# saidwivedi/TokenHMR

Measured on NVIDIA H100. Metric: images/sec (256x192) at bs=64 per GPU, full TokenHMR forward, higher is better.
Workload: dtype f16 operands / f32 accumulate

## Files before the change

### tokenhmr_b200/_build.py

```python
from __future__ import annotations

import hashlib
import os
import subprocess
import sys
from pathlib import Path

PKG_DIR = Path(__file__).resolve().parent
CSRC = PKG_DIR / "csrc"
LIB_PATH = PKG_DIR / "libtokenhmr_b200.so"
STAMP = PKG_DIR / ".libtokenhmr_b200.stamp"
PROBE_SRC = PKG_DIR.parent / "tests" / "csrc" / "kernel_probe.cu"
PROBE_PATH = PKG_DIR.parent / "tests" / "libthmr_probe.so"
PROBE_STAMP = PKG_DIR.parent / "tests" / ".libthmr_probe.stamp"
GEMM_PROBE_SRC = PKG_DIR.parent / "tests" / "csrc" / "gemm_probe.cu"
GEMM_PROBE_PATH = PKG_DIR.parent / "tests" / "libthmr_gemm_probe.so"
GEMM_PROBE_STAMP = PKG_DIR.parent / "tests" / ".libthmr_gemm_probe.stamp"
HEAD_PROBE_SRC = PKG_DIR.parent / "tests" / "csrc" / "head_train_probe.cu"
HEAD_PROBE_PATH = PKG_DIR.parent / "tests" / "libthmr_head_train_probe.so"
HEAD_PROBE_STAMP = PKG_DIR.parent / "tests" / ".libthmr_head_train_probe.stamp"

NVCC_FLAGS = [
    "-gencode", "arch=compute_90a,code=sm_90a",
    "-lineinfo", "-O3", "-std=c++17",
    "--expt-relaxed-constexpr",
    "-Xcompiler", "-fPIC", "-shared",
]
PROBE_FLAGS = ["-Xcompiler", "-fvisibility=hidden"]


def _nvcc() -> str:
    for cand in (os.environ.get("NVCC"), "/usr/local/cuda/bin/nvcc", "nvcc"):
        if cand and (os.path.isabs(cand) and os.path.exists(cand) or not os.path.isabs(cand)):
            return cand
    return "nvcc"


def source_hash(probe: bool = False) -> str:
    h = hashlib.sha256()
    files = sorted(CSRC.glob("*.cu")) + sorted(CSRC.glob("*.cuh")) + sorted((PKG_DIR.parent / "include").glob("*.h"))
    if probe:
        files += sorted(PROBE_SRC.parent.glob("*.cu"))
    for f in files:
        h.update(f.name.encode())
        h.update(f.read_bytes())
    h.update(" ".join(NVCC_FLAGS + (PROBE_FLAGS if probe else [])).encode())
    return h.hexdigest()


def _compile(src: Path, out: Path, stamp: Path, flags: list, want: str, force: bool, verbose: bool) -> Path:
    if not force and out.exists() and stamp.exists() and stamp.read_text().strip() == want:
        return out
    cmd = [_nvcc(), *flags, "-o", str(out), str(src)]
    if verbose:
        cmd.insert(1, "-Xptxas=-v")
        print(" ".join(cmd), file=sys.stderr)
    res = subprocess.run(cmd, capture_output=True, text=True)
    if res.returncode != 0:
        raise RuntimeError(f"nvcc failed ({res.returncode}):\n{res.stdout}\n{res.stderr}")
    if verbose:
        print(res.stderr, file=sys.stderr)
    stamp.write_text(want)
    return out


def build_probe(force: bool = False, verbose: bool = False) -> Path:
    for src, out, stamp in ((GEMM_PROBE_SRC, GEMM_PROBE_PATH, GEMM_PROBE_STAMP),
                            (HEAD_PROBE_SRC, HEAD_PROBE_PATH, HEAD_PROBE_STAMP)):
        if src.exists():
            _compile(src, out, stamp, NVCC_FLAGS + PROBE_FLAGS, source_hash(probe=True), force, verbose)
    return _compile(PROBE_SRC, PROBE_PATH, PROBE_STAMP, NVCC_FLAGS + PROBE_FLAGS, source_hash(probe=True), force,
                    verbose)


def build(force: bool = False, verbose: bool = False) -> Path:
    path = _compile(CSRC / "tokenhmr_b200.cu", LIB_PATH, STAMP, NVCC_FLAGS, source_hash(), force, verbose)
    if PROBE_SRC.exists():
        build_probe(force, verbose)
    return path


if __name__ == "__main__":
    print(build(force="--force" in sys.argv, verbose="-v" in sys.argv))
```

### tokenhmr_b200/csrc/attention_mma.cuh

```cuda
#pragma once
#include "common.cuh"
#include "ptx.cuh"

namespace thmr {

constexpr int kAttTokens = 192;
constexpr int kAttHeadDim = 80;
constexpr int kAttPitch = 88;
constexpr int kAttWarps = 6;
constexpr int kAttThreads = 32 * kAttWarps;
constexpr uint32_t kAttMatBytes = kAttTokens * kAttPitch * 2;
constexpr uint32_t kAttSmemBytes = 3 * kAttMatBytes;

struct AttnParams {
  const __half* qkv;
  int ldq;
  int num_problems;
  int heads;
  float scale_log2e;
  __half* out;
  int ldo;
  float* dbg_s;
  unsigned long long* stamp;
};

__device__ __forceinline__ float fast_exp2(float x) {
  float y;
  asm("ex2.approx.ftz.f32 %0, %1;" : "=f"(y) : "f"(x));
  return y;
}
__device__ __forceinline__ void ldmatrix_x4(uint32_t (&r)[4], uint32_t addr) {
  asm volatile("ldmatrix.sync.aligned.m8n8.x4.shared.b16 {%0, %1, %2, %3}, [%4];"
               : "=r"(r[0]), "=r"(r[1]), "=r"(r[2]), "=r"(r[3]) : "r"(addr));
}
__device__ __forceinline__ void ldmatrix_x4_trans(uint32_t (&r)[4], uint32_t addr) {
  asm volatile("ldmatrix.sync.aligned.m8n8.x4.trans.shared.b16 {%0, %1, %2, %3}, [%4];"
               : "=r"(r[0]), "=r"(r[1]), "=r"(r[2]), "=r"(r[3]) : "r"(addr));
}
__device__ __forceinline__ void mma_16816(float (&d)[4], const uint32_t (&a)[4], uint32_t b0, uint32_t b1) {
  asm volatile("mma.sync.aligned.m16n8k16.row.col.f32.f16.f16.f32 {%0, %1, %2, %3}, {%4, %5, %6, %7}, {%8, %9}, "
               "{%0, %1, %2, %3};"
               : "+f"(d[0]), "+f"(d[1]), "+f"(d[2]), "+f"(d[3])
               : "r"(a[0]), "r"(a[1]), "r"(a[2]), "r"(a[3]), "r"(b0), "r"(b1));
}
__device__ __forceinline__ uint32_t pack_half2(float a, float b) {
  __half2 h = __floats2half2_rn(a, b);
  return *reinterpret_cast<uint32_t*>(&h);
}

template <bool DBG>
__global__ void __launch_bounds__(kAttThreads, 2) vit_attention_kernel(const AttnParams p) {
  extern __shared__ __align__(16) uint8_t att_smem[];
  const uint32_t aQ = smem_u32(att_smem), aK = aQ + kAttMatBytes, aV = aK + kAttMatBytes;
  const int prob = blockIdx.x;
  const int b = prob / p.heads, h = prob % p.heads;
  const int warp = threadIdx.x >> 5, lane = threadIdx.x & 31;

  pdl_launch_dependents();
  stamp_start(p.stamp);
  pdl_wait();

  const __half* src = p.qkv + static_cast<size_t>(b) * kAttTokens * p.ldq;
  for (int i = threadIdx.x; i < 3 * kAttTokens * 10; i += kAttThreads) {
    const int m = i / (kAttTokens * 10), r = (i / 10) % kAttTokens, c = i % 10;
    const __half* g = src + static_cast<size_t>(r) * p.ldq + (m * p.heads + h) * kAttHeadDim + c * 8;
    const uint32_t s = aQ + m * kAttMatBytes + (r * kAttPitch + c * 8) * 2;
    asm volatile("cp.async.cg.shared.global [%0], [%1], 16;" ::"r"(s), "l"(g) : "memory");
  }
  asm volatile("cp.async.commit_group;\n\tcp.async.wait_group 0;" ::: "memory");
  __syncthreads();

  const int g = lane >> 2, t4 = lane & 3;
  for (int tile = warp; tile < kAttTokens / 16; tile += kAttWarps) {
    const int r0 = tile * 16;
    uint32_t qa[5][4];
#pragma unroll
    for (int kk = 0; kk < 5; ++kk)
      ldmatrix_x4(qa[kk], aQ + ((r0 + (lane & 15)) * kAttPitch + kk * 16 + 8 * (lane >> 4)) * 2);
    float s[24][4];
#pragma unroll
    for (int nt = 0; nt < 24; ++nt) s[nt][0] = s[nt][1] = s[nt][2] = s[nt][3] = 0.f;
#pragma unroll
    for (int np = 0; np < 12; ++np) {
#pragma unroll
      for (int kk = 0; kk < 5; ++kk) {
        uint32_t kb[4];
        ldmatrix_x4(kb, aK + ((np * 16 + (lane & 7) + 8 * (lane >> 4)) * kAttPitch + kk * 16 + 8 * ((lane >> 3) & 1)) * 2);
        mma_16816(s[2 * np], qa[kk], kb[0], kb[1]);
        mma_16816(s[2 * np + 1], qa[kk], kb[2], kb[3]);
      }
    }
    if (DBG) {
      float* d = p.dbg_s + (static_cast<size_t>(prob) * kAttTokens + r0 + g) * kAttTokens + 2 * t4;
#pragma unroll
      for (int nt = 0; nt < 24; ++nt) {
        *reinterpret_cast<float2*>(d + nt * 8) = make_float2(s[nt][0], s[nt][1]);
        *reinterpret_cast<float2*>(d + 8 * kAttTokens + nt * 8) = make_float2(s[nt][2], s[nt][3]);
      }
    }
    float mx0 = -INFINITY, mx1 = -INFINITY;
#pragma unroll
    for (int nt = 0; nt < 24; ++nt) {
      mx0 = fmaxf(mx0, fmaxf(s[nt][0], s[nt][1]));
      mx1 = fmaxf(mx1, fmaxf(s[nt][2], s[nt][3]));
    }
#pragma unroll
    for (int off = 1; off <= 2; off <<= 1) {
      mx0 = fmaxf(mx0, __shfl_xor_sync(0xffffffffu, mx0, off));
      mx1 = fmaxf(mx1, __shfl_xor_sync(0xffffffffu, mx1, off));
    }
    const float mo0 = mx0 * p.scale_log2e, mo1 = mx1 * p.scale_log2e;
    float sum0 = 0.f, sum1 = 0.f;
    uint32_t pa[12][4];
#pragma unroll
    for (int nt = 0; nt < 24; ++nt) {
      const float e0 = fast_exp2(fmaf(s[nt][0], p.scale_log2e, -mo0));
      const float e1 = fast_exp2(fmaf(s[nt][1], p.scale_log2e, -mo0));
      const float e2 = fast_exp2(fmaf(s[nt][2], p.scale_log2e, -mo1));
      const float e3 = fast_exp2(fmaf(s[nt][3], p.scale_log2e, -mo1));
      sum0 += e0 + e1;
      sum1 += e2 + e3;
      pa[nt >> 1][(nt & 1) * 2 + 0] = pack_half2(e0, e1);
      pa[nt >> 1][(nt & 1) * 2 + 1] = pack_half2(e2, e3);
    }
#pragma unroll
    for (int off = 1; off <= 2; off <<= 1) {
      sum0 += __shfl_xor_sync(0xffffffffu, sum0, off);
      sum1 += __shfl_xor_sync(0xffffffffu, sum1, off);
    }
    float o[10][4];
#pragma unroll
    for (int dt = 0; dt < 10; ++dt) o[dt][0] = o[dt][1] = o[dt][2] = o[dt][3] = 0.f;
#pragma unroll
    for (int ks = 0; ks < 12; ++ks) {
#pragma unroll
      for (int dp = 0; dp < 5; ++dp) {
        uint32_t vb[4];
        ldmatrix_x4_trans(vb, aV + ((ks * 16 + (lane & 7) + 8 * ((lane >> 3) & 1)) * kAttPitch + dp * 16 + 8 * (lane >> 4)) * 2);
        mma_16816(o[2 * dp], pa[ks], vb[0], vb[1]);
        mma_16816(o[2 * dp + 1], pa[ks], vb[2], vb[3]);
      }
    }
    const float inv0 = 1.0f / sum0, inv1 = 1.0f / sum1;
    __half* out = p.out + (static_cast<size_t>(b) * kAttTokens + r0 + g) * p.ldo + h * kAttHeadDim + 2 * t4;
#pragma unroll
    for (int dt = 0; dt < 10; ++dt) {
      *reinterpret_cast<uint32_t*>(out + dt * 8) = pack_half2(o[dt][0] * inv0, o[dt][1] * inv0);
      *reinterpret_cast<uint32_t*>(out + 8 * static_cast<size_t>(p.ldo) + dt * 8) = pack_half2(o[dt][2] * inv1, o[dt][3] * inv1);
    }
  }
}

struct AttnPlan {
  AttnParams p;
  int grid;
};

inline int attention_make_plan(const __half* qkv, int ld_qkv, int B, int heads, __half* out, int ldo, float* dbg_s,
                               AttnPlan* plan) {
  THMR_CHECK(B > 0 && heads > 0, "attention: bad shape");
  THMR_CHECK(ld_qkv >= 3 * heads * kAttHeadDim, "attention: qkv pitch %d < %d", ld_qkv, 3 * heads * kAttHeadDim);
  THMR_CHECK((reinterpret_cast<uintptr_t>(qkv) & 15) == 0 && ld_qkv % 8 == 0, "attention: qkv pointer/pitch alignment");
  THMR_CHECK(ldo % 2 == 0 && (reinterpret_cast<uintptr_t>(out) & 3) == 0, "attention: output alignment");
  plan->p.qkv = qkv;
  plan->p.ldq = ld_qkv;
  plan->p.num_problems = B * heads;
  plan->p.heads = heads;
  plan->p.scale_log2e = 1.4426950408889634f / sqrtf(static_cast<float>(kAttHeadDim));
  plan->p.out = out;
  plan->p.ldo = ldo;
  plan->p.dbg_s = dbg_s;
  plan->p.stamp = nullptr;
  plan->grid = plan->p.num_problems;
  return THMR_OK;
}

template <bool DBG>
inline int attention_launch_t(const AttnPlan& plan, cudaStream_t st) {
  static bool configured = false;
  if (!configured) {
    THMR_CUDA(cudaFuncSetAttribute(vit_attention_kernel<DBG>, cudaFuncAttributeMaxDynamicSharedMemorySize, kAttSmemBytes));
    configured = true;
  }
  THMR_CUDA(launch_pdl(vit_attention_kernel<DBG>, plan.grid, kAttThreads, kAttSmemBytes, st, plan.p));
  return THMR_OK;
}

inline int attention_dispatch(const AttnPlan& plan, cudaStream_t st) {
  return plan.p.dbg_s ? attention_launch_t<true>(plan, st) : attention_launch_t<false>(plan, st);
}

}
```

### tokenhmr_b200/csrc/ptx.cuh

```cuda
#pragma once
#include <cuda.h>
#include <cuda_fp16.h>
#include <cuda_runtime.h>
#include <stdint.h>

namespace thmr {

__device__ unsigned int g_pipeline_timeout = 0;
constexpr uint32_t kSpinLimit = 1u << 24;

__device__ __forceinline__ uint32_t smem_u32(const void* p) {
  return static_cast<uint32_t>(__cvta_generic_to_shared(p));
}

__device__ __forceinline__ void sts_f32x2(uint32_t a, float x, float y) {
  asm volatile("st.shared.v2.f32 [%0], {%1, %2};" ::"r"(a), "f"(x), "f"(y));
}
__device__ __forceinline__ float4 lds_f32x4(uint32_t a) {
  float4 v;
  asm volatile("ld.shared.v4.f32 {%0, %1, %2, %3}, [%4];" : "=f"(v.x), "=f"(v.y), "=f"(v.z), "=f"(v.w) : "r"(a));
  return v;
}
__device__ __forceinline__ void sts_f32(uint32_t a, float x) { asm volatile("st.shared.f32 [%0], %1;" ::"r"(a), "f"(x)); }
__device__ __forceinline__ void sts_u32(uint32_t a, uint32_t x) { asm volatile("st.shared.b32 [%0], %1;" ::"r"(a), "r"(x)); }
__device__ __forceinline__ float lds_f32(uint32_t a) {
  float v;
  asm volatile("ld.shared.f32 %0, [%1];" : "=f"(v) : "r"(a));
  return v;
}
__device__ __forceinline__ void named_barrier_sync(uint32_t id, uint32_t threads) {
  asm volatile("bar.sync %0, %1;" ::"r"(id), "r"(threads) : "memory");
}

__device__ __forceinline__ unsigned long long globaltimer() {
  unsigned long long t;
  asm volatile("mov.u64 %0, %%globaltimer;" : "=l"(t));
  return t;
}
__device__ __forceinline__ uint32_t smid() {
  uint32_t s;
  asm volatile("mov.u32 %0, %%smid;" : "=r"(s));
  return s;
}

__device__ __forceinline__ uint32_t lane_id() {
  uint32_t l;
  asm volatile("mov.u32 %0, %%laneid;" : "=r"(l));
  return l;
}

__device__ __forceinline__ void mbar_init(uint64_t* bar, uint32_t count) {
  asm volatile("mbarrier.init.shared::cta.b64 [%0], %1;" ::"r"(smem_u32(bar)), "r"(count) : "memory");
}
__device__ __forceinline__ void fence_mbar_init() {
  asm volatile("fence.mbarrier_init.release.cluster;" ::: "memory");
}
__device__ __forceinline__ void fence_proxy_async_smem() {
  asm volatile("fence.proxy.async.shared::cta;" ::: "memory");
}
__device__ __forceinline__ void mbar_arrive(uint64_t* bar) {
  asm volatile("mbarrier.arrive.shared::cta.b64 _, [%0];" ::"r"(smem_u32(bar)) : "memory");
}
__device__ __forceinline__ void mbar_arrive_expect_tx(uint64_t* bar, uint32_t bytes) {
  asm volatile("mbarrier.arrive.expect_tx.shared::cta.b64 _, [%0], %1;" ::"r"(smem_u32(bar)), "r"(bytes)
               : "memory");
}
__device__ __forceinline__ bool mbar_try_wait(uint64_t* bar, uint32_t parity) {
  uint32_t ok;
  asm volatile(
      "{\n\t"
      ".reg .pred P;\n\t"
      "mbarrier.try_wait.parity.shared::cta.b64 P, [%1], %2;\n\t"
      "selp.u32 %0, 1, 0, P;\n\t"
      "}\n"
      : "=r"(ok)
      : "r"(smem_u32(bar)), "r"(parity)
      : "memory");
  return ok != 0;
}
__device__ __forceinline__ bool mbar_wait(uint64_t* bar, uint32_t parity) {
#pragma unroll 1
  for (uint32_t it = 0; it < kSpinLimit; ++it) {
    if (mbar_try_wait(bar, parity)) return true;
  }
  atomicExch(&g_pipeline_timeout, 1u);
  return false;
}

__device__ __forceinline__ uint32_t cluster_ctarank() {
  uint32_t r;
  asm volatile("mov.u32 %0, %%cluster_ctarank;" : "=r"(r));
  return r;
}
__device__ __forceinline__ void cluster_sync_all() {
  asm volatile("barrier.cluster.arrive.release;\n\tbarrier.cluster.wait.acquire;" ::: "memory");
}
__device__ __forceinline__ void mbar_arrive_cluster(uint64_t* bar, uint32_t cta) {
  asm volatile(
      "{\n\t"
      ".reg .b32 ra;\n\t"
      "mapa.shared::cluster.u32 ra, %0, %1;\n\t"
      "mbarrier.arrive.release.cluster.shared::cluster.b64 _, [ra];\n\t"
      "}\n" ::"r"(smem_u32(bar)),
      "r"(cta)
      : "memory");
}
__device__ __forceinline__ bool mbar_wait_cluster(uint64_t* bar, uint32_t parity) {
#pragma unroll 1
  for (uint32_t it = 0; it < kSpinLimit; ++it) {
    uint32_t ok;
    asm volatile(
        "{\n\t"
        ".reg .pred P;\n\t"
        "mbarrier.try_wait.parity.acquire.cluster.shared::cta.b64 P, [%1], %2;\n\t"
        "selp.u32 %0, 1, 0, P;\n\t"
        "}\n"
        : "=r"(ok)
        : "r"(smem_u32(bar)), "r"(parity)
        : "memory");
    if (ok) return true;
  }
  atomicExch(&g_pipeline_timeout, 1u);
  return false;
}

__device__ __forceinline__ void tma_prefetch_desc(const CUtensorMap* m) {
  asm volatile("prefetch.tensormap [%0];" ::"l"(reinterpret_cast<uint64_t>(m)) : "memory");
}
__device__ __forceinline__ void tma_load_2d(void* smem_dst, const CUtensorMap* m, uint64_t* bar, int32_t c0,
                                            int32_t c1) {
  asm volatile(
      "cp.async.bulk.tensor.2d.shared::cluster.global.mbarrier::complete_tx::bytes"
      " [%0], [%1, {%3, %4}], [%2];"
      :
      : "r"(smem_u32(smem_dst)), "l"(reinterpret_cast<uint64_t>(m)), "r"(smem_u32(bar)), "r"(c0), "r"(c1)
      : "memory");
}
__device__ __forceinline__ void tma_load_2d_mcast(void* smem_dst, const CUtensorMap* m, uint64_t* bar, int32_t c0,
                                                  int32_t c1, uint16_t cta_mask) {
  asm volatile(
      "cp.async.bulk.tensor.2d.shared::cluster.global.mbarrier::complete_tx::bytes.multicast::cluster"
      " [%0], [%1, {%3, %4}], [%2], %5;"
      :
      : "r"(smem_u32(smem_dst)), "l"(reinterpret_cast<uint64_t>(m)), "r"(smem_u32(bar)), "r"(c0), "r"(c1),
        "h"(cta_mask)
      : "memory");
}
__device__ __forceinline__ void tma_store_2d(const CUtensorMap* m, uint32_t smem_src, int32_t c0, int32_t c1) {
  asm volatile("cp.async.bulk.tensor.2d.global.shared::cta.bulk_group [%0, {%2, %3}], [%1];"
               :
               : "l"(reinterpret_cast<uint64_t>(m)), "r"(smem_src), "r"(c0), "r"(c1)
               : "memory");
}
__device__ __forceinline__ void tma_reduce_add_2d(const CUtensorMap* m, uint32_t smem_src, int32_t c0, int32_t c1) {
  asm volatile("cp.reduce.async.bulk.tensor.2d.global.shared::cta.add.tile.bulk_group [%0, {%2, %3}], [%1];"
               :
               : "l"(reinterpret_cast<uint64_t>(m)), "r"(smem_src), "r"(c0), "r"(c1)
               : "memory");
}
__device__ __forceinline__ void tma_store_commit() { asm volatile("cp.async.bulk.commit_group;" ::: "memory"); }
template <int N>
__device__ __forceinline__ void tma_store_wait_read() {
  asm volatile("cp.async.bulk.wait_group.read %0;" ::"n"(N) : "memory");
}
template <int N>
__device__ __forceinline__ void tma_store_wait() {
  asm volatile("cp.async.bulk.wait_group %0;" ::"n"(N) : "memory");
}

__device__ __forceinline__ uint64_t make_wgmma_desc_sw128(uint32_t saddr) {
  uint64_t d = 0;
  d |= static_cast<uint64_t>((saddr >> 4) & 0x3FFF);
  d |= static_cast<uint64_t>(1) << 16;
  d |= static_cast<uint64_t>(1024 >> 4) << 32;
  d |= static_cast<uint64_t>(1) << 62;
  return d;
}
__device__ __forceinline__ void wgmma_fence() { asm volatile("wgmma.fence.sync.aligned;" ::: "memory"); }
__device__ __forceinline__ void wgmma_commit() { asm volatile("wgmma.commit_group.sync.aligned;" ::: "memory"); }
template <int N>
__device__ __forceinline__ void wgmma_wait() {
  asm volatile("wgmma.wait_group.sync.aligned %0;" ::"n"(N) : "memory");
}
template <int N>
__device__ __forceinline__ void wgmma_fence_operand(float (&d)[N]) {
#pragma unroll
  for (int i = 0; i < N; ++i) asm volatile("" : "+f"(d[i])::"memory");
}

__device__ __forceinline__ void wgmma_m64n32k16(float (&d)[16], uint64_t da, uint64_t db, uint32_t scale_d) {
  asm volatile(
      "{\n\t.reg .pred p;\n\tsetp.ne.b32 p, %18, 0;\n\t"
      "wgmma.mma_async.sync.aligned.m64n32k16.f32.f16.f16 {%0, %1, %2, %3, %4, %5, %6, %7, %8, %9, %10, %11, %12, %13, %14, %15}, %16, %17, p, 1, 1, 0, 0;\n\t}\n"
      : "+f"(d[0]), "+f"(d[1]), "+f"(d[2]), "+f"(d[3]), "+f"(d[4]), "+f"(d[5]), "+f"(d[6]), "+f"(d[7]), "+f"(d[8]), "+f"(d[9]), "+f"(d[10]), "+f"(d[11]), "+f"(d[12]), "+f"(d[13]), "+f"(d[14]), "+f"(d[15])
      : "l"(da), "l"(db), "r"(scale_d));
}
__device__ __forceinline__ void wgmma_m64n64k16(float (&d)[32], uint64_t da, uint64_t db, uint32_t scale_d) {
  asm volatile(
      "{\n\t.reg .pred p;\n\tsetp.ne.b32 p, %34, 0;\n\t"
      "wgmma.mma_async.sync.aligned.m64n64k16.f32.f16.f16 {%0, %1, %2, %3, %4, %5, %6, %7, %8, %9, %10, %11, %12, %13, %14, %15, %16, %17, %18, %19, %20, %21, %22, %23, %24, %25, %26, %27, %28, %29, %30, %31}, %32, %33, p, 1, 1, 0, 0;\n\t}\n"
      : "+f"(d[0]), "+f"(d[1]), "+f"(d[2]), "+f"(d[3]), "+f"(d[4]), "+f"(d[5]), "+f"(d[6]), "+f"(d[7]), "+f"(d[8]), "+f"(d[9]), "+f"(d[10]), "+f"(d[11]), "+f"(d[12]), "+f"(d[13]), "+f"(d[14]), "+f"(d[15]), "+f"(d[16]), "+f"(d[17]), "+f"(d[18]), "+f"(d[19]), "+f"(d[20]), "+f"(d[21]), "+f"(d[22]), "+f"(d[23]), "+f"(d[24]), "+f"(d[25]), "+f"(d[26]), "+f"(d[27]), "+f"(d[28]), "+f"(d[29]), "+f"(d[30]), "+f"(d[31])
      : "l"(da), "l"(db), "r"(scale_d));
}
__device__ __forceinline__ void wgmma_m64n128k16(float (&d)[64], uint64_t da, uint64_t db, uint32_t scale_d) {
  asm volatile(
      "{\n\t.reg .pred p;\n\tsetp.ne.b32 p, %66, 0;\n\t"
      "wgmma.mma_async.sync.aligned.m64n128k16.f32.f16.f16 {%0, %1, %2, %3, %4, %5, %6, %7, %8, %9, %10, %11, %12, %13, %14, %15, %16, %17, %18, %19, %20, %21, %22, %23, %24, %25, %26, %27, %28, %29, %30, %31, %32, %33, %34, %35, %36, %37, %38, %39, %40, %41, %42, %43, %44, %45, %46, %47, %48, %49, %50, %51, %52, %53, %54, %55, %56, %57, %58, %59, %60, %61, %62, %63}, %64, %65, p, 1, 1, 0, 0;\n\t}\n"
      : "+f"(d[0]), "+f"(d[1]), "+f"(d[2]), "+f"(d[3]), "+f"(d[4]), "+f"(d[5]), "+f"(d[6]), "+f"(d[7]), "+f"(d[8]), "+f"(d[9]), "+f"(d[10]), "+f"(d[11]), "+f"(d[12]), "+f"(d[13]), "+f"(d[14]), "+f"(d[15]), "+f"(d[16]), "+f"(d[17]), "+f"(d[18]), "+f"(d[19]), "+f"(d[20]), "+f"(d[21]), "+f"(d[22]), "+f"(d[23]), "+f"(d[24]), "+f"(d[25]), "+f"(d[26]), "+f"(d[27]), "+f"(d[28]), "+f"(d[29]), "+f"(d[30]), "+f"(d[31]), "+f"(d[32]), "+f"(d[33]), "+f"(d[34]), "+f"(d[35]), "+f"(d[36]), "+f"(d[37]), "+f"(d[38]), "+f"(d[39]), "+f"(d[40]), "+f"(d[41]), "+f"(d[42]), "+f"(d[43]), "+f"(d[44]), "+f"(d[45]), "+f"(d[46]), "+f"(d[47]), "+f"(d[48]), "+f"(d[49]), "+f"(d[50]), "+f"(d[51]), "+f"(d[52]), "+f"(d[53]), "+f"(d[54]), "+f"(d[55]), "+f"(d[56]), "+f"(d[57]), "+f"(d[58]), "+f"(d[59]), "+f"(d[60]), "+f"(d[61]), "+f"(d[62]), "+f"(d[63])
      : "l"(da), "l"(db), "r"(scale_d));
}
__device__ __forceinline__ void wgmma_m64n256k16(float (&d)[128], uint64_t da, uint64_t db, uint32_t scale_d) {
  asm volatile(
      "{\n\t.reg .pred p;\n\tsetp.ne.b32 p, %130, 0;\n\t"
      "wgmma.mma_async.sync.aligned.m64n256k16.f32.f16.f16 {%0, %1, %2, %3, %4, %5, %6, %7, %8, %9, %10, %11, %12, %13, %14, %15, %16, %17, %18, %19, %20, %21, %22, %23, %24, %25, %26, %27, %28, %29, %30, %31, %32, %33, %34, %35, %36, %37, %38, %39, %40, %41, %42, %43, %44, %45, %46, %47, %48, %49, %50, %51, %52, %53, %54, %55, %56, %57, %58, %59, %60, %61, %62, %63, %64, %65, %66, %67, %68, %69, %70, %71, %72, %73, %74, %75, %76, %77, %78, %79, %80, %81, %82, %83, %84, %85, %86, %87, %88, %89, %90, %91, %92, %93, %94, %95, %96, %97, %98, %99, %100, %101, %102, %103, %104, %105, %106, %107, %108, %109, %110, %111, %112, %113, %114, %115, %116, %117, %118, %119, %120, %121, %122, %123, %124, %125, %126, %127}, %128, %129, p, 1, 1, 0, 0;\n\t}\n"
      : "+f"(d[0]), "+f"(d[1]), "+f"(d[2]), "+f"(d[3]), "+f"(d[4]), "+f"(d[5]), "+f"(d[6]), "+f"(d[7]), "+f"(d[8]), "+f"(d[9]), "+f"(d[10]), "+f"(d[11]), "+f"(d[12]), "+f"(d[13]), "+f"(d[14]), "+f"(d[15]), "+f"(d[16]), "+f"(d[17]), "+f"(d[18]), "+f"(d[19]), "+f"(d[20]), "+f"(d[21]), "+f"(d[22]), "+f"(d[23]), "+f"(d[24]), "+f"(d[25]), "+f"(d[26]), "+f"(d[27]), "+f"(d[28]), "+f"(d[29]), "+f"(d[30]), "+f"(d[31]), "+f"(d[32]), "+f"(d[33]), "+f"(d[34]), "+f"(d[35]), "+f"(d[36]), "+f"(d[37]), "+f"(d[38]), "+f"(d[39]), "+f"(d[40]), "+f"(d[41]), "+f"(d[42]), "+f"(d[43]), "+f"(d[44]), "+f"(d[45]), "+f"(d[46]), "+f"(d[47]), "+f"(d[48]), "+f"(d[49]), "+f"(d[50]), "+f"(d[51]), "+f"(d[52]), "+f"(d[53]), "+f"(d[54]), "+f"(d[55]), "+f"(d[56]), "+f"(d[57]), "+f"(d[58]), "+f"(d[59]), "+f"(d[60]), "+f"(d[61]), "+f"(d[62]), "+f"(d[63]), "+f"(d[64]), "+f"(d[65]), "+f"(d[66]), "+f"(d[67]), "+f"(d[68]), "+f"(d[69]), "+f"(d[70]), "+f"(d[71]), "+f"(d[72]), "+f"(d[73]), "+f"(d[74]), "+f"(d[75]), "+f"(d[76]), "+f"(d[77]), "+f"(d[78]), "+f"(d[79]), "+f"(d[80]), "+f"(d[81]), "+f"(d[82]), "+f"(d[83]), "+f"(d[84]), "+f"(d[85]), "+f"(d[86]), "+f"(d[87]), "+f"(d[88]), "+f"(d[89]), "+f"(d[90]), "+f"(d[91]), "+f"(d[92]), "+f"(d[93]), "+f"(d[94]), "+f"(d[95]), "+f"(d[96]), "+f"(d[97]), "+f"(d[98]), "+f"(d[99]), "+f"(d[100]), "+f"(d[101]), "+f"(d[102]), "+f"(d[103]), "+f"(d[104]), "+f"(d[105]), "+f"(d[106]), "+f"(d[107]), "+f"(d[108]), "+f"(d[109]), "+f"(d[110]), "+f"(d[111]), "+f"(d[112]), "+f"(d[113]), "+f"(d[114]), "+f"(d[115]), "+f"(d[116]), "+f"(d[117]), "+f"(d[118]), "+f"(d[119]), "+f"(d[120]), "+f"(d[121]), "+f"(d[122]), "+f"(d[123]), "+f"(d[124]), "+f"(d[125]), "+f"(d[126]), "+f"(d[127])
      : "l"(da), "l"(db), "r"(scale_d));
}

__device__ __forceinline__ void wgmma_m64n64k32_e4m3(float (&d)[32], uint64_t da, uint64_t db, uint32_t scale_d) {
  asm volatile(
      "{\n\t.reg .pred p;\n\tsetp.ne.b32 p, %34, 0;\n\t"
      "wgmma.mma_async.sync.aligned.m64n64k32.f32.e4m3.e4m3 {%0, %1, %2, %3, %4, %5, %6, %7, %8, %9, %10, %11, %12, %13, %14, %15, %16, %17, %18, %19, %20, %21, %22, %23, %24, %25, %26, %27, %28, %29, %30, %31}, %32, %33, p, 1, 1;\n\t}\n"
      : "+f"(d[0]), "+f"(d[1]), "+f"(d[2]), "+f"(d[3]), "+f"(d[4]), "+f"(d[5]), "+f"(d[6]), "+f"(d[7]), "+f"(d[8]), "+f"(d[9]), "+f"(d[10]), "+f"(d[11]), "+f"(d[12]), "+f"(d[13]), "+f"(d[14]), "+f"(d[15]), "+f"(d[16]), "+f"(d[17]), "+f"(d[18]), "+f"(d[19]), "+f"(d[20]), "+f"(d[21]), "+f"(d[22]), "+f"(d[23]), "+f"(d[24]), "+f"(d[25]), "+f"(d[26]), "+f"(d[27]), "+f"(d[28]), "+f"(d[29]), "+f"(d[30]), "+f"(d[31])
      : "l"(da), "l"(db), "r"(scale_d));
}
__device__ __forceinline__ void wgmma_m64n128k32_e4m3(float (&d)[64], uint64_t da, uint64_t db, uint32_t scale_d) {
  asm volatile(
      "{\n\t.reg .pred p;\n\tsetp.ne.b32 p, %66, 0;\n\t"
      "wgmma.mma_async.sync.aligned.m64n128k32.f32.e4m3.e4m3 {%0, %1, %2, %3, %4, %5, %6, %7, %8, %9, %10, %11, %12, %13, %14, %15, %16, %17, %18, %19, %20, %21, %22, %23, %24, %25, %26, %27, %28, %29, %30, %31, %32, %33, %34, %35, %36, %37, %38, %39, %40, %41, %42, %43, %44, %45, %46, %47, %48, %49, %50, %51, %52, %53, %54, %55, %56, %57, %58, %59, %60, %61, %62, %63}, %64, %65, p, 1, 1;\n\t}\n"
      : "+f"(d[0]), "+f"(d[1]), "+f"(d[2]), "+f"(d[3]), "+f"(d[4]), "+f"(d[5]), "+f"(d[6]), "+f"(d[7]), "+f"(d[8]), "+f"(d[9]), "+f"(d[10]), "+f"(d[11]), "+f"(d[12]), "+f"(d[13]), "+f"(d[14]), "+f"(d[15]), "+f"(d[16]), "+f"(d[17]), "+f"(d[18]), "+f"(d[19]), "+f"(d[20]), "+f"(d[21]), "+f"(d[22]), "+f"(d[23]), "+f"(d[24]), "+f"(d[25]), "+f"(d[26]), "+f"(d[27]), "+f"(d[28]), "+f"(d[29]), "+f"(d[30]), "+f"(d[31]), "+f"(d[32]), "+f"(d[33]), "+f"(d[34]), "+f"(d[35]), "+f"(d[36]), "+f"(d[37]), "+f"(d[38]), "+f"(d[39]), "+f"(d[40]), "+f"(d[41]), "+f"(d[42]), "+f"(d[43]), "+f"(d[44]), "+f"(d[45]), "+f"(d[46]), "+f"(d[47]), "+f"(d[48]), "+f"(d[49]), "+f"(d[50]), "+f"(d[51]), "+f"(d[52]), "+f"(d[53]), "+f"(d[54]), "+f"(d[55]), "+f"(d[56]), "+f"(d[57]), "+f"(d[58]), "+f"(d[59]), "+f"(d[60]), "+f"(d[61]), "+f"(d[62]), "+f"(d[63])
      : "l"(da), "l"(db), "r"(scale_d));
}

__device__ __forceinline__ uint16_t cvt_e4m3x2(float lo, float hi) {
  uint16_t r;
  asm("cvt.rn.satfinite.e4m3x2.f32 %0, %1, %2;" : "=h"(r) : "f"(hi), "f"(lo));
  return r;
}

__device__ __forceinline__ float e4m3_scale(float amax) {
  if (!(amax > 0.f)) return 1.0f;
  int E;
  const float m = frexpf(amax, &E);
  return ldexpf(1.0f, m <= 0.875f ? E - 9 : E - 8);
}

__device__ __forceinline__ void bulk_load_1d(void* smem_dst, const void* src, uint32_t bytes, uint64_t* bar) {
  asm volatile("cp.async.bulk.shared::cluster.global.mbarrier::complete_tx::bytes [%0], [%1], %2, [%3];"
               :
               : "r"(smem_u32(smem_dst)), "l"(reinterpret_cast<uint64_t>(src)), "r"(bytes), "r"(smem_u32(bar))
               : "memory");
}

}
```

Measured before the change: 1894.

## Port ViT attention to persistent WGMMA kernel with double-buffered TMA loads

Rewrites the per-head attention kernel to use Hopper warpgroup MMA (SS for QK^T, register-sourced for PV) instead of mma.sync with ldmatrix. Q/K/V tiles are loaded by TMA with swizzled layouts, split into a 64-column wide part and a 16-column tail, and double-buffered across problems in a persistent grid sized to the SM count. The aim is to cut instruction overhead and overlap the next head's loads with the current compute. In exchange, occupancy drops to one 384-thread block per SM, and the kernel becomes more complex, relying on descriptor and barrier correctness.

```diff
diff --git a/tokenhmr_b200/_build.py b/tokenhmr_b200/_build.py
--- a/tokenhmr_b200/_build.py
+++ b/tokenhmr_b200/_build.py
@@ -19,6 +19,9 @@
 HEAD_PROBE_SRC = PKG_DIR.parent / "tests" / "csrc" / "head_train_probe.cu"
 HEAD_PROBE_PATH = PKG_DIR.parent / "tests" / "libthmr_head_train_probe.so"
 HEAD_PROBE_STAMP = PKG_DIR.parent / "tests" / ".libthmr_head_train_probe.stamp"
+ATT_PROBE_SRC = PKG_DIR.parent / "tests" / "csrc" / "attention_probe.cu"
+ATT_PROBE_PATH = PKG_DIR.parent / "tests" / "libthmr_attention_probe.so"
+ATT_PROBE_STAMP = PKG_DIR.parent / "tests" / ".libthmr_attention_probe.stamp"
 
 NVCC_FLAGS = [
     "-gencode", "arch=compute_90a,code=sm_90a",
@@ -66,7 +69,8 @@
 
 def build_probe(force: bool = False, verbose: bool = False) -> Path:
     for src, out, stamp in ((GEMM_PROBE_SRC, GEMM_PROBE_PATH, GEMM_PROBE_STAMP),
-                            (HEAD_PROBE_SRC, HEAD_PROBE_PATH, HEAD_PROBE_STAMP)):
+                            (HEAD_PROBE_SRC, HEAD_PROBE_PATH, HEAD_PROBE_STAMP),
+                            (ATT_PROBE_SRC, ATT_PROBE_PATH, ATT_PROBE_STAMP)):
         if src.exists():
             _compile(src, out, stamp, NVCC_FLAGS + PROBE_FLAGS, source_hash(probe=True), force, verbose)
     return _compile(PROBE_SRC, PROBE_PATH, PROBE_STAMP, NVCC_FLAGS + PROBE_FLAGS, source_hash(probe=True), force,
diff --git a/tokenhmr_b200/csrc/attention_mma.cuh b/tokenhmr_b200/csrc/attention_mma.cuh
--- a/tokenhmr_b200/csrc/attention_mma.cuh
+++ b/tokenhmr_b200/csrc/attention_mma.cuh
@@ -6,11 +6,13 @@
 
 constexpr int kAttTokens = 192;
 constexpr int kAttHeadDim = 80;
-constexpr int kAttPitch = 88;
-constexpr int kAttWarps = 6;
-constexpr int kAttThreads = 32 * kAttWarps;
-constexpr uint32_t kAttMatBytes = kAttTokens * kAttPitch * 2;
-constexpr uint32_t kAttSmemBytes = 3 * kAttMatBytes;
+constexpr int kAttWarpgroups = 3;
+constexpr int kAttThreads = 128 * kAttWarpgroups;
+constexpr uint32_t kAttWideBytes = kAttTokens * 128;
+constexpr uint32_t kAttTailBytes = kAttTokens * 32;
+constexpr uint32_t kAttHeadBytes = 3 * (kAttWideBytes + kAttTailBytes);
+constexpr int kAttBufs = 2;
+constexpr uint32_t kAttSmemBytes = kAttBufs * kAttHeadBytes + 3 * kAttBufs * 8 + 1024;
 
 struct AttnParams {
   const __half* qkv;
@@ -29,80 +31,88 @@
   asm("ex2.approx.ftz.f32 %0, %1;" : "=f"(y) : "f"(x));
   return y;
 }
-__device__ __forceinline__ void ldmatrix_x4(uint32_t (&r)[4], uint32_t addr) {
-  asm volatile("ldmatrix.sync.aligned.m8n8.x4.shared.b16 {%0, %1, %2, %3}, [%4];"
-               : "=r"(r[0]), "=r"(r[1]), "=r"(r[2]), "=r"(r[3]) : "r"(addr));
-}
-__device__ __forceinline__ void ldmatrix_x4_trans(uint32_t (&r)[4], uint32_t addr) {
-  asm volatile("ldmatrix.sync.aligned.m8n8.x4.trans.shared.b16 {%0, %1, %2, %3}, [%4];"
-               : "=r"(r[0]), "=r"(r[1]), "=r"(r[2]), "=r"(r[3]) : "r"(addr));
-}
-__device__ __forceinline__ void mma_16816(float (&d)[4], const uint32_t (&a)[4], uint32_t b0, uint32_t b1) {
-  asm volatile("mma.sync.aligned.m16n8k16.row.col.f32.f16.f16.f32 {%0, %1, %2, %3}, {%4, %5, %6, %7}, {%8, %9}, "
-               "{%0, %1, %2, %3};"
-               : "+f"(d[0]), "+f"(d[1]), "+f"(d[2]), "+f"(d[3])
-               : "r"(a[0]), "r"(a[1]), "r"(a[2]), "r"(a[3]), "r"(b0), "r"(b1));
-}
 __device__ __forceinline__ uint32_t pack_half2(float a, float b) {
   __half2 h = __floats2half2_rn(a, b);
   return *reinterpret_cast<uint32_t*>(&h);
 }
 
+__device__ __forceinline__ void attention_issue_loads(const CUtensorMap* tm_wide, const CUtensorMap* tm_tail,
+                                                      uint8_t* buf, uint64_t* full, int prob, int heads) {
+  const int b = prob / heads, h = prob % heads;
+  const int row = b * kAttTokens;
+  mbar_arrive_expect_tx(&full[0], 2 * (kAttWideBytes + kAttTailBytes));
+  mbar_arrive_expect_tx(&full[1], kAttWideBytes + kAttTailBytes);
+#pragma unroll
+  for (int m = 0; m < 3; ++m) {
+    const int col = (m * heads + h) * kAttHeadDim;
+    uint64_t* bar = &full[m == 2 ? 1 : 0];
+    tma_load_2d(buf + m * kAttWideBytes, tm_wide, bar, col, row);
+    tma_load_2d(buf + 3 * kAttWideBytes + m * kAttTailBytes, tm_tail, bar, col + 64, row);
+  }
+}
+
 template <bool DBG>
-__global__ void __launch_bounds__(kAttThreads, 2) vit_attention_kernel(const AttnParams p) {
-  extern __shared__ __align__(16) uint8_t att_smem[];
-  const uint32_t aQ = smem_u32(att_smem), aK = aQ + kAttMatBytes, aV = aK + kAttMatBytes;
-  const int prob = blockIdx.x;
-  const int b = prob / p.heads, h = prob % p.heads;
-  const int warp = threadIdx.x >> 5, lane = threadIdx.x & 31;
-
+__global__ void __launch_bounds__(kAttThreads, 1)
+vit_attention_kernel(const __grid_constant__ CUtensorMap tm_wide, const __grid_constant__ CUtensorMap tm_tail,
+                     const AttnParams p) {
+  extern __shared__ __align__(1024) uint8_t att_smem_raw[];
+  uint8_t* smem = reinterpret_cast<uint8_t*>((reinterpret_cast<uintptr_t>(att_smem_raw) + 1023) & ~uintptr_t(1023));
+  uint64_t* bars = reinterpret_cast<uint64_t*>(smem + kAttBufs * kAttHeadBytes);
+  unsigned int* done = reinterpret_cast<unsigned int*>(bars + 2 * kAttBufs);
+  const int wg = threadIdx.x >> 7, warp = (threadIdx.x >> 5) & 3, lane = threadIdx.x & 31;
+  const int g = lane >> 2, t4 = lane & 3;
+
+  if (threadIdx.x == 0) {
+    tma_prefetch_desc(&tm_wide);
+    tma_prefetch_desc(&tm_tail);
+    for (int i = 0; i < 2 * kAttBufs; ++i) mbar_init(&bars[i], 1);
+    for (int i = 0; i < kAttBufs; ++i) done[i] = 0;
+    fence_mbar_init();
+  }
+  __syncthreads();
   pdl_launch_dependents();
   stamp_start(p.stamp);
   pdl_wait();
 
-  const __half* src = p.qkv + static_cast<size_t>(b) * kAttTokens * p.ldq;
-  for (int i = threadIdx.x; i < 3 * kAttTokens * 10; i += kAttThreads) {
-    const int m = i / (kAttTokens * 10), r = (i / 10) % kAttTokens, c = i % 10;
-    const __half* g = src + static_cast<size_t>(r) * p.ldq + (m * p.heads + h) * kAttHeadDim + c * 8;
-    const uint32_t s = aQ + m * kAttMatBytes + (r * kAttPitch + c * 8) * 2;
-    asm volatile("cp.async.cg.shared.global [%0], [%1], 16;" ::"r"(s), "l"(g) : "memory");
-  }
-  asm volatile("cp.async.commit_group;\n\tcp.async.wait_group 0;" ::: "memory");
-  __syncthreads();
-
-  const int g = lane >> 2, t4 = lane & 3;
-  for (int tile = warp; tile < kAttTokens / 16; tile += kAttWarps) {
-    const int r0 = tile * 16;
-    uint32_t qa[5][4];
-#pragma unroll
-    for (int kk = 0; kk < 5; ++kk)
-      ldmatrix_x4(qa[kk], aQ + ((r0 + (lane & 15)) * kAttPitch + kk * 16 + 8 * (lane >> 4)) * 2);
-    float s[24][4];
-#pragma unroll
-    for (int nt = 0; nt < 24; ++nt) s[nt][0] = s[nt][1] = s[nt][2] = s[nt][3] = 0.f;
-#pragma unroll
-    for (int np = 0; np < 12; ++np) {
-#pragma unroll
-      for (int kk = 0; kk < 5; ++kk) {
-        uint32_t kb[4];
-        ldmatrix_x4(kb, aK + ((np * 16 + (lane & 7) + 8 * (lane >> 4)) * kAttPitch + kk * 16 + 8 * ((lane >> 3) & 1)) * 2);
-        mma_16816(s[2 * np], qa[kk], kb[0], kb[1]);
-        mma_16816(s[2 * np + 1], qa[kk], kb[2], kb[3]);
-      }
-    }
+  if (threadIdx.x == 0) {
+    for (int i = 0; i < kAttBufs && blockIdx.x + i * gridDim.x < p.num_problems; ++i)
+      attention_issue_loads(&tm_wide, &tm_tail, smem + i * kAttHeadBytes, bars + 2 * i, blockIdx.x + i * gridDim.x,
+                            p.heads);
+  }
+
+  int it = 0;
+  for (int prob = blockIdx.x; prob < p.num_problems; prob += gridDim.x, ++it) {
+    const int buf = it % kAttBufs;
+    const uint32_t parity = (it / kAttBufs) & 1;
+    uint64_t* full = bars + 2 * buf;
+    const uint32_t sQ = smem_u32(smem + buf * kAttHeadBytes), sK = sQ + kAttWideBytes, sV = sK + kAttWideBytes;
+    const uint32_t tQ = sQ + 3 * kAttWideBytes, tK = tQ + kAttTailBytes, tV = tK + kAttTailBytes;
+    const int b = prob / p.heads, h = prob % p.heads;
+    const int r0 = wg * 64 + warp * 16;
+
+    mbar_wait(&full[0], parity);
+    float s[96];
+    wgmma_fence();
+#pragma unroll
+    for (int kk = 0; kk < 4; ++kk)
+      wgmma_m64n192k16(s, make_wgmma_desc_sw128(sQ + wg * 64 * 128 + kk * 32), make_wgmma_desc_sw128(sK + kk * 32), kk);
+    wgmma_m64n192k16(s, make_wgmma_desc(tQ + wg * 64 * 32, 16, 256, 3), make_wgmma_desc(tK, 16, 256, 3), 1);
+    wgmma_commit();
+    wgmma_wait<0>();
+    wgmma_fence_operand(s);
     if (DBG) {
       float* d = p.dbg_s + (static_cast<size_t>(prob) * kAttTokens + r0 + g) * kAttTokens + 2 * t4;
 #pragma unroll
       for (int nt = 0; nt < 24; ++nt) {
-        *reinterpret_cast<float2*>(d + nt * 8) = make_float2(s[nt][0], s[nt][1]);
-        *reinterpret_cast<float2*>(d + 8 * kAttTokens + nt * 8) = make_float2(s[nt][2], s[nt][3]);
+        *reinterpret_cast<float2*>(d + nt * 8) = make_float2(s[4 * nt], s[4 * nt + 1]);
+        *reinterpret_cast<float2*>(d + 8 * kAttTokens + nt * 8) = make_float2(s[4 * nt + 2], s[4 * nt + 3]);
       }
     }
     float mx0 = -INFINITY, mx1 = -INFINITY;
 #pragma unroll
     for (int nt = 0; nt < 24; ++nt) {
-      mx0 = fmaxf(mx0, fmaxf(s[nt][0], s[nt][1]));
-      mx1 = fmaxf(mx1, fmaxf(s[nt][2], s[nt][3]));
+      mx0 = fmaxf(mx0, fmaxf(s[4 * nt], s[4 * nt + 1]));
+      mx1 = fmaxf(mx1, fmaxf(s[4 * nt + 2], s[4 * nt + 3]));
     }
 #pragma unroll
     for (int off = 1; off <= 2; off <<= 1) {
@@ -114,10 +124,10 @@
     uint32_t pa[12][4];
 #pragma unroll
     for (int nt = 0; nt < 24; ++nt) {
-      const float e0 = fast_exp2(fmaf(s[nt][0], p.scale_log2e, -mo0));
-      const float e1 = fast_exp2(fmaf(s[nt][1], p.scale_log2e, -mo0));
-      const float e2 = fast_exp2(fmaf(s[nt][2], p.scale_log2e, -mo1));
-      const float e3 = fast_exp2(fmaf(s[nt][3], p.scale_log2e, -mo1));
+      const float e0 = fast_exp2(fmaf(s[4 * nt + 0], p.scale_log2e, -mo0));
+      const float e1 = fast_exp2(fmaf(s[4 * nt + 1], p.scale_log2e, -mo0));
+      const float e2 = fast_exp2(fmaf(s[4 * nt + 2], p.scale_log2e, -mo1));
+      const float e3 = fast_exp2(fmaf(s[4 * nt + 3], p.scale_log2e, -mo1));
       sum0 += e0 + e1;
       sum1 += e2 + e3;
       pa[nt >> 1][(nt & 1) * 2 + 0] = pack_half2(e0, e1);
@@ -128,30 +138,40 @@
       sum0 += __shfl_xor_sync(0xffffffffu, sum0, off);
       sum1 += __shfl_xor_sync(0xffffffffu, sum1, off);
     }
-    float o[10][4];
-#pragma unroll
-    for (int dt = 0; dt < 10; ++dt) o[dt][0] = o[dt][1] = o[dt][2] = o[dt][3] = 0.f;
+    mbar_wait(&full[1], parity);
+    float o[32], ot[8];
+    wgmma_fence();
 #pragma unroll
     for (int ks = 0; ks < 12; ++ks) {
-#pragma unroll
-      for (int dp = 0; dp < 5; ++dp) {
-        uint32_t vb[4];
-        ldmatrix_x4_trans(vb, aV + ((ks * 16 + (lane & 7) + 8 * ((lane >> 3) & 1)) * kAttPitch + dp * 16 + 8 * (lane >> 4)) * 2);
-        mma_16816(o[2 * dp], pa[ks], vb[0], vb[1]);
-        mma_16816(o[2 * dp + 1], pa[ks], vb[2], vb[3]);
+      wgmma_m64n64k16_rs_tb(o, pa[ks], make_wgmma_desc(sV + ks * 16 * 128, 1024, 1024, 1), ks);
+      wgmma_m64n16k16_rs_tb(ot, pa[ks], make_wgmma_desc(tV + ks * 16 * 32, 256, 256, 3), ks);
+    }
+    wgmma_commit();
+    wgmma_wait<0>();
+    wgmma_fence_operand(o);
+    wgmma_fence_operand(ot);
+    named_barrier_sync(1 + wg, 128);
+    if ((threadIdx.x & 127) == 0 && prob + kAttBufs * static_cast<int>(gridDim.x) < p.num_problems) {
+      __threadfence_block();
+      if (atomicAdd(&done[buf], 1u) == kAttWarpgroups - 1) {
+        done[buf] = 0;
+        __threadfence_block();
+        attention_issue_loads(&tm_wide, &tm_tail, smem + buf * kAttHeadBytes, full, prob + kAttBufs * gridDim.x, p.heads);
       }
     }
     const float inv0 = 1.0f / sum0, inv1 = 1.0f / sum1;
     __half* out = p.out + (static_cast<size_t>(b) * kAttTokens + r0 + g) * p.ldo + h * kAttHeadDim + 2 * t4;
 #pragma unroll
     for (int dt = 0; dt < 10; ++dt) {
-      *reinterpret_cast<uint32_t*>(out + dt * 8) = pack_half2(o[dt][0] * inv0, o[dt][1] * inv0);
-      *reinterpret_cast<uint32_t*>(out + 8 * static_cast<size_t>(p.ldo) + dt * 8) = pack_half2(o[dt][2] * inv1, o[dt][3] * inv1);
+      const float* c = dt < 8 ? &o[4 * dt] : &ot[4 * (dt - 8)];
+      *reinterpret_cast<uint32_t*>(out + dt * 8) = pack_half2(c[0] * inv0, c[1] * inv0);
+      *reinterpret_cast<uint32_t*>(out + 8 * static_cast<size_t>(p.ldo) + dt * 8) = pack_half2(c[2] * inv1, c[3] * inv1);
     }
   }
 }
 
 struct AttnPlan {
+  CUtensorMap tm_wide, tm_tail;
   AttnParams p;
   int grid;
 };
@@ -162,6 +182,9 @@
   THMR_CHECK(ld_qkv >= 3 * heads * kAttHeadDim, "attention: qkv pitch %d < %d", ld_qkv, 3 * heads * kAttHeadDim);
   THMR_CHECK((reinterpret_cast<uintptr_t>(qkv) & 15) == 0 && ld_qkv % 8 == 0, "attention: qkv pointer/pitch alignment");
   THMR_CHECK(ldo % 2 == 0 && (reinterpret_cast<uintptr_t>(out) & 3) == 0, "attention: output alignment");
+  const uint64_t rows = static_cast<uint64_t>(B) * kAttTokens, cols = 3ull * heads * kAttHeadDim;
+  THMR_TRY(make_tmap_2d_f16(&plan->tm_wide, qkv, rows, cols, ld_qkv, kAttTokens, 64, CU_TENSOR_MAP_SWIZZLE_128B));
+  THMR_TRY(make_tmap_2d_f16(&plan->tm_tail, qkv, rows, cols, ld_qkv, kAttTokens, 16, CU_TENSOR_MAP_SWIZZLE_32B));
   plan->p.qkv = qkv;
   plan->p.ldq = ld_qkv;
   plan->p.num_problems = B * heads;
@@ -171,7 +194,7 @@
   plan->p.ldo = ldo;
   plan->p.dbg_s = dbg_s;
   plan->p.stamp = nullptr;
-  plan->grid = plan->p.num_problems;
+  plan->grid = plan->p.num_problems < num_sms() ? plan->p.num_problems : num_sms();
   return THMR_OK;
 }
 
@@ -182,7 +205,8 @@
     THMR_CUDA(cudaFuncSetAttribute(vit_attention_kernel<DBG>, cudaFuncAttributeMaxDynamicSharedMemorySize, kAttSmemBytes));
     configured = true;
   }
-  THMR_CUDA(launch_pdl(vit_attention_kernel<DBG>, plan.grid, kAttThreads, kAttSmemBytes, st, plan.p));
+  THMR_CUDA(launch_pdl(vit_attention_kernel<DBG>, plan.grid, kAttThreads, kAttSmemBytes, st, plan.tm_wide, plan.tm_tail,
+                       plan.p));
   return THMR_OK;
 }
 
diff --git a/tokenhmr_b200/csrc/ptx.cuh b/tokenhmr_b200/csrc/ptx.cuh
--- a/tokenhmr_b200/csrc/ptx.cuh
+++ b/tokenhmr_b200/csrc/ptx.cuh
@@ -176,6 +176,14 @@
   d |= static_cast<uint64_t>(1) << 62;
   return d;
 }
+__device__ __forceinline__ uint64_t make_wgmma_desc(uint32_t saddr, uint32_t lbo, uint32_t sbo, uint32_t layout) {
+  uint64_t d = 0;
+  d |= static_cast<uint64_t>((saddr >> 4) & 0x3FFF);
+  d |= static_cast<uint64_t>((lbo >> 4) & 0x3FFF) << 16;
+  d |= static_cast<uint64_t>((sbo >> 4) & 0x3FFF) << 32;
+  d |= static_cast<uint64_t>(layout) << 62;
+  return d;
+}
 __device__ __forceinline__ void wgmma_fence() { asm volatile("wgmma.fence.sync.aligned;" ::: "memory"); }
 __device__ __forceinline__ void wgmma_commit() { asm volatile("wgmma.commit_group.sync.aligned;" ::: "memory"); }
 template <int N>
@@ -216,6 +224,29 @@
       : "+f"(d[0]), "+f"(d[1]), "+f"(d[2]), "+f"(d[3]), "+f"(d[4]), "+f"(d[5]), "+f"(d[6]), "+f"(d[7]), "+f"(d[8]), "+f"(d[9]), "+f"(d[10]), "+f"(d[11]), "+f"(d[12]), "+f"(d[13]), "+f"(d[14]), "+f"(d[15]), "+f"(d[16]), "+f"(d[17]), "+f"(d[18]), "+f"(d[19]), "+f"(d[20]), "+f"(d[21]), "+f"(d[22]), "+f"(d[23]), "+f"(d[24]), "+f"(d[25]), "+f"(d[26]), "+f"(d[27]), "+f"(d[28]), "+f"(d[29]), "+f"(d[30]), "+f"(d[31]), "+f"(d[32]), "+f"(d[33]), "+f"(d[34]), "+f"(d[35]), "+f"(d[36]), "+f"(d[37]), "+f"(d[38]), "+f"(d[39]), "+f"(d[40]), "+f"(d[41]), "+f"(d[42]), "+f"(d[43]), "+f"(d[44]), "+f"(d[45]), "+f"(d[46]), "+f"(d[47]), "+f"(d[48]), "+f"(d[49]), "+f"(d[50]), "+f"(d[51]), "+f"(d[52]), "+f"(d[53]), "+f"(d[54]), "+f"(d[55]), "+f"(d[56]), "+f"(d[57]), "+f"(d[58]), "+f"(d[59]), "+f"(d[60]), "+f"(d[61]), "+f"(d[62]), "+f"(d[63]), "+f"(d[64]), "+f"(d[65]), "+f"(d[66]), "+f"(d[67]), "+f"(d[68]), "+f"(d[69]), "+f"(d[70]), "+f"(d[71]), "+f"(d[72]), "+f"(d[73]), "+f"(d[74]), "+f"(d[75]), "+f"(d[76]), "+f"(d[77]), "+f"(d[78]), "+f"(d[79]), "+f"(d[80]), "+f"(d[81]), "+f"(d[82]), "+f"(d[83]), "+f"(d[84]), "+f"(d[85]), "+f"(d[86]), "+f"(d[87]), "+f"(d[88]), "+f"(d[89]), "+f"(d[90]), "+f"(d[91]), "+f"(d[92]), "+f"(d[93]), "+f"(d[94]), "+f"(d[95]), "+f"(d[96]), "+f"(d[97]), "+f"(d[98]), "+f"(d[99]), "+f"(d[100]), "+f"(d[101]), "+f"(d[102]), "+f"(d[103]), "+f"(d[104]), "+f"(d[105]), "+f"(d[106]), "+f"(d[107]), "+f"(d[108]), "+f"(d[109]), "+f"(d[110]), "+f"(d[111]), "+f"(d[112]), "+f"(d[113]), "+f"(d[114]), "+f"(d[115]), "+f"(d[116]), "+f"(d[117]), "+f"(d[118]), "+f"(d[119]), "+f"(d[120]), "+f"(d[121]), "+f"(d[122]), "+f"(d[123]), "+f"(d[124]), "+f"(d[125]), "+f"(d[126]), "+f"(d[127])
       : "l"(da), "l"(db), "r"(scale_d));
 }
+
+__device__ __forceinline__ void wgmma_m64n192k16(float (&d)[96], uint64_t da, uint64_t db, uint32_t scale_d) {
+  asm volatile(
+      "{\n\t.reg .pred p;\n\tsetp.ne.b32 p, %98, 0;\n\t"
+      "wgmma.mma_async.sync.aligned.m64n192k16.f32.f16.f16 {%0, %1, %2, %3, %4, %5, %6, %7, %8, %9, %10, %11, %12, %13, %14, %15, %16, %17, %18, %19, %20, %21, %22, %23, %24, %25, %26, %27, %28, %29, %30, %31, %32, %33, %34, %35, %36, %37, %38, %39, %40, %41, %42, %43, %44, %45, %46, %47, %48, %49, %50, %51, %52, %53, %54, %55, %56, %57, %58, %59, %60, %61, %62, %63, %64, %65, %66, %67, %68, %69, %70, %71, %72, %73, %74, %75, %76, %77, %78, %79, %80, %81, %82, %83, %84, %85, %86, %87, %88, %89, %90, %91, %92, %93, %94, %95}, %96, %97, p, 1, 1, 0, 0;\n\t}\n"
+      : "+f"(d[0]), "+f"(d[1]), "+f"(d[2]), "+f"(d[3]), "+f"(d[4]), "+f"(d[5]), "+f"(d[6]), "+f"(d[7]), "+f"(d[8]), "+f"(d[9]), "+f"(d[10]), "+f"(d[11]), "+f"(d[12]), "+f"(d[13]), "+f"(d[14]), "+f"(d[15]), "+f"(d[16]), "+f"(d[17]), "+f"(d[18]), "+f"(d[19]), "+f"(d[20]), "+f"(d[21]), "+f"(d[22]), "+f"(d[23]), "+f"(d[24]), "+f"(d[25]), "+f"(d[26]), "+f"(d[27]), "+f"(d[28]), "+f"(d[29]), "+f"(d[30]), "+f"(d[31]), "+f"(d[32]), "+f"(d[33]), "+f"(d[34]), "+f"(d[35]), "+f"(d[36]), "+f"(d[37]), "+f"(d[38]), "+f"(d[39]), "+f"(d[40]), "+f"(d[41]), "+f"(d[42]), "+f"(d[43]), "+f"(d[44]), "+f"(d[45]), "+f"(d[46]), "+f"(d[47]), "+f"(d[48]), "+f"(d[49]), "+f"(d[50]), "+f"(d[51]), "+f"(d[52]), "+f"(d[53]), "+f"(d[54]), "+f"(d[55]), "+f"(d[56]), "+f"(d[57]), "+f"(d[58]), "+f"(d[59]), "+f"(d[60]), "+f"(d[61]), "+f"(d[62]), "+f"(d[63]), "+f"(d[64]), "+f"(d[65]), "+f"(d[66]), "+f"(d[67]), "+f"(d[68]), "+f"(d[69]), "+f"(d[70]), "+f"(d[71]), "+f"(d[72]), "+f"(d[73]), "+f"(d[74]), "+f"(d[75]), "+f"(d[76]), "+f"(d[77]), "+f"(d[78]), "+f"(d[79]), "+f"(d[80]), "+f"(d[81]), "+f"(d[82]), "+f"(d[83]), "+f"(d[84]), "+f"(d[85]), "+f"(d[86]), "+f"(d[87]), "+f"(d[88]), "+f"(d[89]), "+f"(d[90]), "+f"(d[91]), "+f"(d[92]), "+f"(d[93]), "+f"(d[94]), "+f"(d[95])
+      : "l"(da), "l"(db), "r"(scale_d));
+}
+__device__ __forceinline__ void wgmma_m64n64k16_rs_tb(float (&d)[32], const uint32_t (&a)[4], uint64_t db, uint32_t scale_d) {
+  asm volatile(
+      "{\n\t.reg .pred p;\n\tsetp.ne.b32 p, %37, 0;\n\t"
+      "wgmma.mma_async.sync.aligned.m64n64k16.f32.f16.f16 {%0, %1, %2, %3, %4, %5, %6, %7, %8, %9, %10, %11, %12, %13, %14, %15, %16, %17, %18, %19, %20, %21, %22, %23, %24, %25, %26, %27, %28, %29, %30, %31}, {%32, %33, %34, %35}, %36, p, 1, 1, 1;\n\t}\n"
+      : "+f"(d[0]), "+f"(d[1]), "+f"(d[2]), "+f"(d[3]), "+f"(d[4]), "+f"(d[5]), "+f"(d[6]), "+f"(d[7]), "+f"(d[8]), "+f"(d[9]), "+f"(d[10]), "+f"(d[11]), "+f"(d[12]), "+f"(d[13]), "+f"(d[14]), "+f"(d[15]), "+f"(d[16]), "+f"(d[17]), "+f"(d[18]), "+f"(d[19]), "+f"(d[20]), "+f"(d[21]), "+f"(d[22]), "+f"(d[23]), "+f"(d[24]), "+f"(d[25]), "+f"(d[26]), "+f"(d[27]), "+f"(d[28]), "+f"(d[29]), "+f"(d[30]), "+f"(d[31])
+      : "r"(a[0]), "r"(a[1]), "r"(a[2]), "r"(a[3]), "l"(db), "r"(scale_d));
+}
+__device__ __forceinline__ void wgmma_m64n16k16_rs_tb(float (&d)[8], const uint32_t (&a)[4], uint64_t db, uint32_t scale_d) {
+  asm volatile(
+      "{\n\t.reg .pred p;\n\tsetp.ne.b32 p, %13, 0;\n\t"
+      "wgmma.mma_async.sync.aligned.m64n16k16.f32.f16.f16 {%0, %1, %2, %3, %4, %5, %6, %7}, {%8, %9, %10, %11}, %12, p, 1, 1, 1;\n\t}\n"
+      : "+f"(d[0]), "+f"(d[1]), "+f"(d[2]), "+f"(d[3]), "+f"(d[4]), "+f"(d[5]), "+f"(d[6]), "+f"(d[7])
+      : "r"(a[0]), "r"(a[1]), "r"(a[2]), "r"(a[3]), "l"(db), "r"(scale_d));
+}
+
 
 __device__ __forceinline__ void wgmma_m64n64k32_e4m3(float (&d)[32], uint64_t da, uint64_t db, uint32_t scale_d) {
   asm volatile(
```

Measured after the change: 1928, median of 6. No clear change (+1.8%).
